# gargatik/Seamless-Through-Breaking-Rethinking-Image-Stitching-for-Optimal-Alignment

Measured on AMD Instinct MI355X. Metric: stitched image-pairs/s at 512x512, higher is better.
Workload: dtype f32 (decoder contractions, PatchEmbed's third conv and the C = 128 block tails: exact 3xbf16 split of both operands, 6 products on the bf16 matrix cores, fp32 accumulate -- error vs fp64 0.83x the fp32 MFMA chain's; everything else fp32); 1 GPU; UDIS-D-shaped 512x512 pairs, batch=1, FlowHomoAdpater.forward(type=test_eval); launch=hipGraph replay, pairs_in_flight=3

## Files before the change

include/stitch_gfx950.h:

```cpp
#ifndef STITCH_GFX950_H
#define STITCH_GFX950_H
#include <stdint.h>
#ifdef __cplusplus
extern "C" {
#endif

typedef struct st_gemm_desc {
    const float* a;
    const float* w;
    float* c;
    const float* bias;
    const float* aux0;
    const float* aux1;
    const float* aux2;
    const float* scale_ptr;
    int32_t M, N, K;
    int32_t H, W, Cin, ldx;
    int32_t kh, kw, sh, sw, ph, pw, Ho, Wo;
    int32_t ldw, ldc, ld_aux0, ld_aux1, ld_aux2;
    int32_t aux0_row_div, aux0_row_mod;
    int32_t act;
    int32_t epi;
    float alpha;
    int32_t batch;
// ... 45 lines not shown
    int32_t ld_res;
    int32_t act;
    int32_t ln;
    float ln_eps;
    int32_t res;
    int32_t res_layer;
} st_chain_layer;
typedef struct st_chain_desc {
    const float* a;
    float* out;
    int32_t lda, ldo, M, nlayers;
    st_chain_layer layer[3];
} st_chain_desc;
int st_linear_chain128(const st_chain_desc* desc, void* stream);
int st_abi_chain_desc_size(void);

typedef struct st_mlp_desc {
    const float* a;
    float* out;
    const float* w1;
    const float* b1;
    const float* w2;
    const float* b2;
    const float* res;
    int32_t lda, ldo, ld_res, M, hidden, ln;
    float ln_eps;
    int32_t reserved;
    const float* wp;
    const float* bp;
    const float* res0;
    int32_t ld_res0, reserved1;
} st_mlp_desc;
int st_mlp128(const st_mlp_desc* desc, void* stream);
int st_abi_mlp_desc_size(void);
int st_mlp128_split3_image_bytes(int32_t hidden, int32_t with_proj, int64_t* bytes);
int st_mlp128_split3_pack(const float* w1, const float* b1, const float* w2, const float* wp, const float* bp, int32_t hidden, void* image,
                          int64_t image_bytes, void* stream);
int st_mlp128_split3(const st_mlp_desc* desc, const void* image, int64_t image_bytes, void* stream);
int st_rowlin128_split3_image_bytes(int32_t N, int64_t* bytes);
int st_rowlin128_split3_pack(const float* w, const float* b, int32_t N, void* image, int64_t image_bytes, void* stream);
int st_rowlin128_split3(const float* a, int32_t lda, float* out, int32_t ldo, int32_t M, int32_t N, int32_t ln, float ln_eps, const void* image,
                        int64_t image_bytes, const float* aux, int32_t ld_aux, int32_t row_div, void* stream);

int st_corr_volume(const float* f1, const float* f2, float* vol, int32_t B, int32_t N1, int32_t N2,
                   int32_t C, void* stream);
int st_corr_volume_both(const float* f1, const float* f2, float* vol12, float* vol21, int32_t B, int32_t N, int32_t C,
                        void* stream);
int st_corr_volume_both_plan(int32_t B, int32_t N, int32_t C, int32_t aligned16);

int st_layernorm(const float* x, int32_t ldx, const float* w, const float* b, float* out, int32_t ldo,
                 int32_t rows, int32_t C, float eps, void* stream);
int st_softmax_rows(float* x, int32_t ld, int32_t rows, int32_t C, void* stream);
int st_l2norm_rows(const float* x, float* out, int32_t rows, int32_t C, void* stream);
int st_maxpool_nhwc(const float* x, float* out, int32_t B, int32_t H, int32_t W, int32_t C, int32_t k,
                    int32_t s, int32_t p, void* stream);
int st_dwconv3x3_residual(const float* x, const float* w, const float* bias, float* out, int32_t B,
                          int32_t H, int32_t W, int32_t C, void* stream);
int st_sine_pe(float* out, int32_t ld, int32_t rows, int32_t dim, const float* coords, int32_t ldc,
               int32_t Wg, int32_t ws, int32_t period, float cscale, float coff, int32_t accumulate,
               void* stream);
int st_attention_small(const float* q, int64_t q_bs, int64_t q_ts, const float* k, int64_t k_bs, int64_t k_ts,
                       const float* v, int64_t v_bs, int64_t v_ts, float* out, int64_t o_bs, int64_t o_ts,
                       int32_t B, int32_t heads, int32_t Nq, int32_t Nk, int32_t D, float scale, void* stream);
int st_attention_kvlds(const float* q, int64_t q_bs, int64_t q_ts, const float* k, int64_t k_bs, int64_t k_ts,
                       const float* v, int64_t v_bs, int64_t v_ts, float* out, int64_t o_bs, int64_t o_ts,
                       int32_t B, int32_t heads, int32_t Nq, int32_t Nk, int32_t D, float scale, void* stream);
int st_window_attention(const float* q, const float* k, const float* v, int64_t bs, int64_t ts,
                        const float* qpad, const float* kpad, const float* vpad, float* out, int64_t o_bs,
                        int64_t o_ts, int32_t B, int32_t H, int32_t W, int32_t heads, int32_t D, int32_t ws,
                        float scale, void* stream);
int st_ccl_softargmax(const float* G, float* out, int32_t ldo, int32_t B, int32_t h, int32_t w, void* stream);
int st_patch_conv1(const float* maps, const float* w36x16, const float* bias, float* out, int32_t M, int32_t H,
                   int32_t W, int32_t Ho, int32_t Wo, void* stream);
int st_patch_conv12(const float* cost_maps, const float* c0_w36x16, const float* c0_b, const float* c2_w32x576,
                    const float* c2_b, float* s2, int32_t M, int32_t H, int32_t W, void* stream);
int st_patch_conv12_planes(const float* cost_maps, const float* c0_w36x16, const float* c0_b, const float* c2_w32x576, const float* c2_b,
                           void* s2_planes, int64_t s2_pstride, int32_t M, int32_t H, int32_t W, void* stream);
int st_copy2d(const float* src, int32_t lds, float* dst, int32_t ldd, int32_t rows, int32_t cols, void* stream);
int st_prep_image(const float* src, float* dst, int32_t B, int32_t C, int32_t H, int32_t W, int32_t ldo,
                  float mul, float div, float sub, void* stream);

int st_latent_pool(const float* scores, int32_t ld_s, const float* tokens, int32_t ld_t, float* z, int32_t pixels,
                   int32_t P, void* stream);

int st_coords_grid(float* out, int32_t B, int32_t H, int32_t W, void* stream);
int st_coords_grid_init(float* out, const float* init, int32_t B, int32_t H, int32_t W, void* stream);
int st_flow_forward_interpolate(const float* src, int32_t src_is_coords_rows, float* out, int32_t B, int32_t H, int32_t W,
                                void* stream);
int st_flow_from_coords(const float* coords1, float* flow4, int32_t ld4, float* dst2, int32_t ld2, int32_t B,
                        int32_t H, int32_t W, void* stream);
int st_flow_encode(const float* coords1, const float* w98, const float* bias, float* out, int32_t ldo, float* flow2,
                   int32_t ld2, int32_t B, int32_t H, int32_t W, int32_t Co, void* stream);
int st_flow_encode_split3(const float* coords1, const float* w98, const float* bias, float* out, int32_t ldo, float* flow2,
                          int32_t ld2, int32_t B, int32_t H, int32_t W, int32_t Co, void* out_planes, int64_t out_pstride,
                          int64_t out_prows, void* flow_planes, int64_t flow_pstride, int64_t flow_prows, int32_t flow_col,
                          void* stream);
int st_cost_lookup(const float* maps, const float* coords, float* out, int32_t ldo, int32_t Nq, int32_t H2,
                   int32_t W2, int32_t r, void* stream);
int st_decoder_token_chain(float* corr, int32_t ld_corr, const float* coords1, const float* kv,
                           const float* const* weights16, int32_t rows, int32_t ntok, void* stream);
int st_convex_upsample(const float* coords1, const float* mask, int32_t ldm, float* out, int32_t B, int32_t H,
                       int32_t W, void* stream);

int st_dlt4(const float* src4x2, const float* motion, float* H, int32_t B, float mscale_x, float mscale_y,
            float div, void* stream);
int st_mat3_sandwich(const float* L, const float* X, const float* R, float* out, int32_t B, int32_t invert,
                     void* stream);
int st_homo_warp(const float* U, const float* theta, float* out, int32_t* idx, int32_t B, int32_t C,
                 int32_t n_ones, int32_t H, int32_t W, int32_t oh, int32_t ow, void* stream);
int st_mesh_bounds(const float* H, float* out4, int32_t B, float width, float height, int32_t gw, int32_t gh,
                   void* stream);
int st_flow_warp(const float* x, const float* flow, const float* mul, float* out, int32_t B, int32_t C,
                 int32_t H, int32_t W, void* stream);
int st_homo_flow_warp(const float* image2, const float* H8, const float* flow, float* out6, float* overlap, float* Hi,
                      int32_t B, int32_t H, int32_t W, void* stream);
int st_resize_bilinear(const float* x, float* out, int32_t planes, int32_t H, int32_t W, int32_t oh, int32_t ow,
                       int32_t align_corners, float div0, float div1, int32_t ndiv, void* stream);
int st_range_map(const float* flow, void* scratch_u64, float* out, int32_t B, int32_t H, int32_t W, void* stream);
int st_occlusion_from_range(const float* range, float* out, int64_t n, int32_t threshold, void* stream);
int st_morph_open(const float* mask, float* out, void* scratch_u8x2, int32_t N, int32_t H, int32_t W,
                  int32_t ksz, void* stream);
int st_eval_finish(float* final6, const float* occ, float* overlap, int32_t B, int32_t H, int32_t W, void* stream);
int st_blend(const float* homo1, const float* homo2, float* fin, const float* occ, float* output2, float* mask1,
             float* mask2, uint8_t* blend, int32_t h, int32_t w, void* stream);
int st_blend_plain(const float* homo1, const float* homo2, const float* fin, float* output2, float* mask1, float* mask2,
                   uint8_t* blend, int32_t h, int32_t w, void* stream);
int st_mean_threshold(const float* x, float* out, int32_t B, int32_t C, int32_t H, int32_t W, float thr,
                      void* stream);
int st_tps_solve_grid(const float* U, const float* source, const float* target, void* work_f64, float* T,
                      float* out, int32_t* idx, int32_t B, int32_t C, int32_t H, int32_t W, int32_t N,
                      int32_t oh, int32_t ow, void* stream);

int st_masked_psnr_ssim(const float* image1, const float* warped, int64_t warped_batch_stride, const float* maskmean,
                        void* partial_f64, double* out_psnr_ssim, int32_t B, int32_t H, int32_t W, void* stream);
int st_channel_mean(const float* x, int64_t batch_stride, float* out, int32_t B, int32_t C, int32_t H, int32_t W,
                    void* stream);

int st_load_rgb8(const void* src_u8_hwc, float* dst_chw, int32_t B, int32_t H, int32_t W, void* stream);

int st_cost_lookup9x9(const float* maps, const float* coords, float* out, int32_t ldo, int32_t Nq, int32_t H2,
                      int32_t W2, void* stream);
int st_grid_sample_blend(const float* x, const float* flow, const float* mul, float* out, int32_t B, int32_t C,
                         int32_t H, int32_t W, void* stream);
int st_morph_open19(const float* mask, float* out, void* scratch_u8x2, int32_t N, int32_t H, int32_t W,
                    void* stream);
int st_patch_embed(const float* cost_maps, const float* const* weights, int32_t ld_f0, const float* pe_bias,
                   float* s1, float* s2, float* s3, float* s4, float* tokens, int32_t M, int32_t H, int32_t W,
                   void* workspace, int64_t workspace_floats, void* stream);
int st_patch_embed_split3(const float* cost_maps, const float* const* weights, int32_t ld_f0, const float* pe_bias, void* s2_planes,
                          int64_t s2_pstride, const void* c4_w_planes, int64_t c4_w_pstride, float* s3, float* s4, float* tokens, int32_t M,
                          int32_t H, int32_t W, const void* tail_image, int64_t tail_image_bytes, void* workspace, int64_t workspace_floats, void* stream);
int st_pe_tail_split3_image_bytes(int64_t* bytes);
int st_pe_tail_split3_pack(const float* w1, int32_t ld1, const float* w2, void* image, int64_t image_bytes, void* stream);
int st_pe_tail_split3(const float* x, const float* tab, int32_t P, const void* image, int64_t image_bytes, const float* b2, const float* gamma,
                      const float* beta, float eps, float* out, int32_t R, void* stream);
int st_gma_attention(const float* inp, int32_t ld_inp, const float* w_qk, float* qk, float* attn, int32_t B,
                     int32_t N, void* workspace, int64_t workspace_floats, void* stream);
int st_gma_aggregate(const float* attn, const float* mf, int32_t ld_mf, const float* w_v, const float* gamma,
                     float* vT, float* out, int32_t ld_out, int32_t B, int32_t N, void* workspace,
                     int64_t workspace_floats, void* stream);
int st_sepconv_gru(float* hxA, float* hxB, int32_t ld, float* zbuf, const float* tab1, const float* tab2,
                   int32_t ld_tab, const float* w_zr1, const float* w_q1, const float* w_zr2, const float* w_q2,
                   int32_t B, int32_t H, int32_t W, void* workspace, int64_t workspace_floats, void* stream);
int st_gma_aggregate_planes(const float* attn, const float* mf, int32_t ld_mf, const float* w_v, const float* gamma, float* vT,
                            float* out, int32_t ld_out, void* out_planes, int64_t out_pstride, int64_t out_prows, int32_t out_col, int32_t B,
                            int32_t N, void* workspace, int64_t workspace_floats, void* stream);
// ... 82 lines not shown
```

seamless-through-breaking-rethinking-image-stitching-for-optimal-alignment_amd/csrc/nn.hip:

```cpp
#include "common.h"
#include "../../include/stitch_gfx950.h"

__global__ __launch_bounds__(256) void layernorm_kernel(const float* __restrict__ x, int ldx, const float* __restrict__ w,
                                                        const float* __restrict__ b, float* __restrict__ out, int ldo,
                                                        int rows, int C, float eps) {
    const int row = (blockIdx.x * 256 + threadIdx.x) >> 6, lane = threadIdx.x & 63;
    if (row >= rows) return;
    const float* xr = x + (size_t)row * ldx;
    float v[16];
    float s = 0.f;
#pragma unroll
    for (int i = 0; i < 16; ++i) {
        const int c = lane + 64 * i;
        v[i] = c < C ? xr[c] : 0.f;
        s += v[i];
    }
    const float mean = wave_sum(s) / (float)C;
    float q = 0.f;
#pragma unroll
    for (int i = 0; i < 16; ++i) {
        const int c = lane + 64 * i;
        const float dlt = c < C ? v[i] - mean : 0.f;
        q += dlt * dlt;
    }
// ... 274 lines not shown
        }
    }
    const float inv = 1.0f / sum;
    float* op = out + b * o_bs + iq * o_ts + h * D;
#pragma unroll
    for (int e = 0; e < D; e += 4)
        *reinterpret_cast<float4*>(op + e) = make_float4(acc[e] * inv, acc[e + 1] * inv, acc[e + 2] * inv, acc[e + 3] * inv);
}

extern "C" int st_attention_small(const float* q, int64_t q_bs, int64_t q_ts, const float* k, int64_t k_bs, int64_t k_ts,
                                  const float* v, int64_t v_bs, int64_t v_ts, float* out, int64_t o_bs, int64_t o_ts,
                                  int32_t B, int32_t heads, int32_t Nq, int32_t Nk, int32_t D, float scale, void* stream) {
    if (!q || !k || !v || !out || B <= 0 || heads <= 0 || Nq <= 0 || Nk <= 0) return ST_EINVAL;
    if (!al16(q) || !al16(k) || !al16(v) || !al16(out) || ((q_bs | q_ts | k_bs | k_ts | v_bs | v_ts | o_bs | o_ts) & 3)) return ST_EINVAL;
    const long total = (long)B * heads * Nq;
    dim3 grid((total + 255) / 256), block(256);
    hipStream_t s = (hipStream_t)stream;
#define LAUNCH_AS(DD) hipLaunchKernelGGL(attention_small_kernel<DD>, grid, block, 0, s, q, q_bs, q_ts, k, k_bs, k_ts, v, \
                                         v_bs, v_ts, out, o_bs, o_ts, B, heads, Nq, Nk, scale)
    if (D == 8) LAUNCH_AS(8); else if (D == 16) LAUNCH_AS(16); else if (D == 32) LAUNCH_AS(32); else return ST_EINVAL;
#undef LAUNCH_AS
    ST_CHECK_LAUNCH();
    return ST_OK;
}

typedef float lp_f32x16 __attribute__((ext_vector_type(16)));

__global__ __launch_bounds__(256) void latent_pool_kernel(const float* __restrict__ scores, int ld_s, const float* __restrict__ tokens,
                                                          int ld_t, float* __restrict__ z, int P) {
    const size_t pix = blockIdx.x;
    const int lane = threadIdx.x & 63, wave = threadIdx.x >> 6;
    const int li = lane & 31, lh = lane >> 5;
    const int ib = wave & 1, jb0 = (wave >> 1) * 2;
    const float* Sp = scores + pix * P * ld_s + ib * 32 + li;
    const float* Tp = tokens + pix * P * ld_t + jb0 * 32 + li;
    const int steps = P >> 1;
    float a[32];
    float mx = -INFINITY;
#pragma unroll
    for (int s = 0; s < 32; ++s) {
        a[s] = s < steps ? Sp[(size_t)(2 * s + lh) * ld_s] : -INFINITY;
        mx = fmaxf(mx, a[s]);
    }
    mx = fmaxf(mx, __shfl_xor(mx, 32, 64));
    float sum = 0.f;
#pragma unroll
    for (int s = 0; s < 32; ++s) { a[s] = __expf(a[s] - mx); sum += a[s]; }
    sum += __shfl_xor(sum, 32, 64);
    const float inv = 1.0f / sum;
    lp_f32x16 acc0, acc1;
#pragma unroll
    for (int r = 0; r < 16; ++r) { acc0[r] = 0.f; acc1[r] = 0.f; }
#pragma unroll
    for (int s0 = 0; s0 < 32; s0 += 8) {
        if (s0 < steps) {
            float b0[8], b1[8];
#pragma unroll
            for (int u = 0; u < 8; ++u) {
                const int tok = min(2 * (s0 + u) + lh, P - 1);
                b0[u] = Tp[(size_t)tok * ld_t];
                b1[u] = Tp[(size_t)tok * ld_t + 32];
            }
#pragma unroll
            for (int u = 0; u < 8; ++u) {
                const float av = a[s0 + u] * inv;
                acc0 = __builtin_amdgcn_mfma_f32_32x32x2f32(av, b0[u], acc0, 0, 0, 0);
                acc1 = __builtin_amdgcn_mfma_f32_32x32x2f32(av, b1[u], acc1, 0, 0, 0);
            }
        }
    }
    float* zp = z + (pix * 64 + ib * 32 + 4 * lh) * 128 + jb0 * 32 + li;
#pragma unroll
    for (int r = 0; r < 16; ++r) {
        const int row = (r & 3) + 8 * (r >> 2);
        zp[(size_t)row * 128] = acc0[r];
        zp[(size_t)row * 128 + 32] = acc1[r];
    }
}

extern "C" int st_latent_pool(const float* scores, int32_t ld_s, const float* tokens, int32_t ld_t, float* z, int32_t pixels,
                              int32_t P, void* stream) {
    if (!scores || !tokens || !z || pixels <= 0 || P <= 0 || (P & 1) || P > 64 || ld_s < 64 || ld_t < 128) return ST_EINVAL;
    hipLaunchKernelGGL(latent_pool_kernel, dim3(pixels), dim3(256), 0, (hipStream_t)stream, scores, ld_s, tokens, ld_t, z, P);
    ST_CHECK_LAUNCH();
    return ST_OK;
}

template <int D>
__global__ __launch_bounds__(256) void attention_kvlds_kernel(const float* __restrict__ q, long q_bs, long q_ts,
                                                              const float* __restrict__ k, long k_bs, long k_ts,
                                                              const float* __restrict__ v, long v_bs, long v_ts,
                                                              float* __restrict__ out, long o_bs, long o_ts, int Nq, int Nk,
                                                              float scale) {
    extern __shared__ __attribute__((aligned(16))) float kv[];
    constexpr int QPT = 2;
    const int h = blockIdx.y, b = blockIdx.z;
    float* Ks = kv;
    float* Vs = kv + (size_t)Nk * D;
    for (int i = threadIdx.x; i < Nk * (D / 4); i += 256) {
        const int j = i / (D / 4), e = (i % (D / 4)) * 4;
        *reinterpret_cast<float4*>(Ks + j * D + e) = *reinterpret_cast<const float4*>(k + b * k_bs + j * k_ts + h * D + e);
        *reinterpret_cast<float4*>(Vs + j * D + e) = *reinterpret_cast<const float4*>(v + b * v_bs + j * v_ts + h * D + e);
    }
    __syncthreads();
    const int iq0 = blockIdx.x * (256 * QPT) + threadIdx.x;
    if (iq0 >= Nq) return;
    float qr[QPT][D], acc[QPT][D], mx[QPT], sum[QPT];
    bool live[QPT];
#pragma unroll
    for (int u = 0; u < QPT; ++u) {
        const int iq = iq0 + 256 * u;
        live[u] = iq < Nq;
        const float* qp = q + b * q_bs + (long)(live[u] ? iq : iq0) * q_ts + h * D;
#pragma unroll
        for (int e = 0; e < D; e += 4) {
            const float4 t = *reinterpret_cast<const float4*>(qp + e);
            qr[u][e] = t.x * scale; qr[u][e + 1] = t.y * scale; qr[u][e + 2] = t.z * scale; qr[u][e + 3] = t.w * scale;
        }
#pragma unroll
        for (int e = 0; e < D; ++e) acc[u][e] = 0.f;
        mx[u] = -INFINITY; sum[u] = 0.f;
    }
    for (int j0 = 0; j0 < Nk; j0 += 8) {
        float s[QPT][8];
#pragma unroll
        for (int jj = 0; jj < 8; ++jj) {
            const int j = j0 + jj;
#pragma unroll
            for (int u = 0; u < QPT; ++u) s[u][jj] = 0.f;
            if (j < Nk) {
#pragma unroll
                for (int e = 0; e < D; e += 4) {
                    const float4 t = *reinterpret_cast<const float4*>(Ks + j * D + e);
#pragma unroll
                    for (int u = 0; u < QPT; ++u) {
                        s[u][jj] = fmaf(qr[u][e], t.x, s[u][jj]); s[u][jj] = fmaf(qr[u][e + 1], t.y, s[u][jj]);
                        s[u][jj] = fmaf(qr[u][e + 2], t.z, s[u][jj]); s[u][jj] = fmaf(qr[u][e + 3], t.w, s[u][jj]);
                    }
                }
            } else {
#pragma unroll
                for (int u = 0; u < QPT; ++u) s[u][jj] = -INFINITY;
            }
        }
#pragma unroll
        for (int u = 0; u < QPT; ++u) {
            float nm = mx[u];
#pragma unroll
            for (int jj = 0; jj < 8; ++jj) nm = fmaxf(nm, s[u][jj]);
            const float corr = __expf(mx[u] - nm);
            mx[u] = nm;
            sum[u] *= corr;
#pragma unroll
            for (int e = 0; e < D; ++e) acc[u][e] *= corr;
#pragma unroll
            for (int jj = 0; jj < 8; ++jj) { s[u][jj] = __expf(s[u][jj] - nm); sum[u] += s[u][jj]; }
        }
#pragma unroll
        for (int jj = 0; jj < 8; ++jj) {
            const int j = j0 + jj;
            if (j < Nk) {
#pragma unroll
                for (int e = 0; e < D; e += 4) {
                    const float4 t = *reinterpret_cast<const float4*>(Vs + j * D + e);
#pragma unroll
                    for (int u = 0; u < QPT; ++u) {
// ... 507 lines not shown
```

seamless-through-breaking-rethinking-image-stitching-for-optimal-alignment_amd/flowformer.py:

```python
from __future__ import annotations

import os

import torch
import torch.nn as nn

from . import ops
from .checkpoint import HP, ParamTree, flat_params, flow_spec
from .homography import pack_conv


SPLIT3 = os.environ.get("ST_SPLIT3", "1") != "0"


def _new(rows, cols, dev, zero=False):
    return (torch.zeros if zero else torch.empty)((rows, cols), device=dev, dtype=torch.float32)


def _planes_copy(p):
    return ops.Planes(p.rows, p.C, None, t=p.t.clone(), c0=p.c0, ncols=p.ncols)


def _keep(trace, **named):
    if trace is None:
# ... 241 lines not shown
            ops.conv_gemm(h, fc2[0], o, bias=fc2[1], aux0=x, epi="add", aux1=extra_res)
        return o

    def _twins(self, t, x, B, H, W, trace=None):
        dev = x.device
        dims, heads, srs, patch = (128, 256), (4, 8), (8, 4), (4, 2)
        for s in range(2):
            C, hd, sr, ps = dims[s], heads[s], srs[s], patch[s]
            H, W = H // ps, W // ps
            N = B * H * W
            e = _new(N, C, dev)
            ops.conv_gemm(x, t[f"pe{s}"][0], e, geom=(B, H * ps, W * ps, ps, ps, ps, ps, 0, 0), bias=t[f"pe{s}"][1])
            x = _new(N, C, dev)
            ops.layernorm(e, t[f"pen{s}"][0], t[f"pen{s}"][1], x, 1e-5)
            L = t[f"l{s}"]
            y = _new(N, C, dev)
            qkv = _new(N, 3 * C, dev)
            if L.get("qkv_s3") is not None:
                ops.rowlin128_split3(x, qkv, L["qkv_s3"], ln_eps=1e-6)
            elif "qkv_ln" in L:
                ops.conv_gemm(x, L["qkv_ln"][0], qkv, bias=L["qkv_ln"][1], ln_eps=1e-6)
            else:
                ops.layernorm(x, L["n1"][0], L["n1"][1], y, 1e-6)
                ops.conv_gemm(y, L["qkv"][0], qkv, bias=L["qkv"][1])
            att = _new(N, C, dev)
            ops.window_attention(qkv[:, :C], qkv[:, C:2 * C], qkv[:, 2 * C:], H * W * 3 * C, 3 * C, *L["pads"], att,
                                 H * W * C, C, B, H, W, hd, C // hd, 7, (C // hd) ** -0.5)
            x2 = self._mlp(att, L["proj"], x, L["n2"], L["fc1"], L["fc2"], 1e-6, fc1_ln=L.get("fc1_ln"), image=L.get("mlp_s3"))
            x3 = _new(N, C, dev)
            ops.dwconv3x3_residual(x2, t[f"peg{s}"][0], t[f"peg{s}"][1], x3, B, H, W, C)
            Gk = t[f"g{s}"]
            ops.layernorm(x3, Gk["n1"][0], Gk["n1"][1], y, 1e-6)
            q = _new(N, C, dev)
            ops.conv_gemm(y, Gk["q"][0], q, bias=Gk["q"][1])
            Hk, Wk = H // sr, W // sr
            Nk = Hk * Wk
            xs = _new(B * Nk, C, dev)
            ops.conv_gemm(y, Gk["sr"][0], xs, geom=(B, H, W, sr, sr, sr, sr, 0, 0), bias=Gk["sr"][1])
            xsn = _new(B * Nk, C, dev)
            ops.layernorm(xs, Gk["srn"][0], Gk["srn"][1], xsn, 1e-5)
            kv = _new(B * Nk, 2 * C, dev)
            ops.conv_gemm(xsn, Gk["kv"][0], kv, bias=Gk["kv"][1])
            ops.attention_kvlds(q, (H * W * C, C), kv[:, :C], (Nk * 2 * C, 2 * C), kv[:, C:], (Nk * 2 * C, 2 * C), att,
                                (H * W * C, C), B, hd, H * W, Nk, C // hd, (C // hd) ** -0.5)
            rec = _record(trace)
            _keep(rec, H=H, W=W, pe=x, lsa=x2, peg=x3)
            x = self._mlp(att, Gk["proj"], x3, Gk["n2"], Gk["fc1"], Gk["fc2"], 1e-6, fc1_ln=Gk.get("fc1_ln"), image=Gk.get("mlp_s3"))
            _keep(rec, gsa=x)
        return x, H, W

    def _patch_embed(self, cost_maps, M, H2, W2):
        pe = self._pk["pe"]
        dev = cost_maps.device
        Hp, Wp = (H2 + 7) // 8 * 8, (W2 + 7) // 8 * 8
        H1, W1, H2p, W2p, h, w = Hp // 2, Wp // 2, Hp // 4, Wp // 4, Hp // 8, Wp // 8
        P = h * w
        key = ("pe_tab", h, w)
        if key not in self._const:
            tab_in = _new(P, 64, dev)
            ops.sine_pe(tab_in, 64, Wg=w, cscale=8.0, coff=4.0)
            tab = _new(P, 128, dev)
            ops.conv_gemm(tab_in, pe["f0"][0][:, 64:], tab, bias=pe["f0"][1])
            self._const[key] = tab
        s3, s4, f = _new(M * P, 64, dev), _new(M * P, 128, dev), _new(M * P, 128, dev)
        if H2 == 64 and W2 == 64 and "c4_s3" in pe:
            CH = 16384
            s2p = ops.Planes(min(M, CH) * 256, 32, dev)
            for m0 in range(0, M, CH):
                m1 = min(M, m0 + CH)
                ops.patch_embed_split3(cost_maps[m0:m1], pe["embed11"], pe["f0"][0].stride(0), self._const[key], s2p, pe["c4_s3"],
                                       s3[m0 * P:m1 * P], s4[m0 * P:m1 * P], f[m0 * P:m1 * P], m1 - m0, H2, W2, tail_image=pe.get("tail_s3"))
            return f, P
        s1 = None if (H2 == 64 and W2 == 64) else _new(M * H1 * W1, 16, dev)
        s2 = _new(M * H2p * W2p, 32, dev)
        ops.patch_embed(cost_maps, pe["embed11"], pe["f0"][0].stride(0), self._const[key], s1, s2, s3, s4, f, M, H2, W2)
        return f, P

    def _latent_input(self, L, tokens, M, P):
        dev = tokens.device
        lat = self._pk["latents"]
        nl = lat.shape[0]
        att = _new(M * nl, 128, dev)
        if nl == 8 and P % 2 == 0 and P <= 64:
            S = _new(M * P, nl * 8, dev)
            ops.conv_gemm(tokens, L["qfold"], S)
            z = _new(M * nl * 8, 128, dev)
            ops.latent_pool(S, tokens, z, M, P)
            ops.conv_gemm(z.view(M * nl, 8 * 128)[:, :128], L["wv_heads"][:16], att[:, :16], batch=8, bsa=128, bsw=16 * 128, bsc=16)
            proj_b = L["proj_b_fold"]
        else:
            qn = _new(nl, 128, dev)
            ops.layernorm(lat, L["n1"][0], L["n1"][1], qn, 1e-5)
            q = _new(nl, 128, dev)
            ops.conv_gemm(qn, L["q"][0], q, bias=L["q"][1])
            kv = _new(M * P, 256, dev)
            ops.conv_gemm(tokens, L["kv"][0], kv, bias=L["kv"][1])
            ops.attention_small(q, (0, 128), kv[:, :128], (P * 256, 256), kv[:, 128:], (P * 256, 256), att, (nl * 128, 128),
                                M, 8, nl, P, 16, 16 ** -0.5)
            proj_b = L["proj"][1]
        x1 = _new(M * nl, 128, dev)
        ops.conv_gemm(att, L["proj"][0], x1, bias=proj_b, aux0=lat, row_mod=nl)
        o = _new(M * nl, 128, dev)
        if L.get("mlp_s3_plain") is not None:
            return ops.mlp128(x1, o, L["f0_ln"][0], L["f0_ln"][1], L["f3"][0], L["f3"][1], ln_eps=1e-5, image=L["mlp_s3_plain"])
        return ops.linear_chain128(x1, o, [dict(w=L["f0_ln"][0], bias=L["f0_ln"][1], act="gelu", ln_eps=1e-5), dict(w=L["f3"][0], bias=L["f3"][1], res=0)])

    def _latent_self(self, L, x, M):
        dev = x.device
        nl = self._pk["latents"].shape[0]
        qkv = _new(M * nl, 384, dev)
        if L.get("qkv_s3") is not None:
            ops.rowlin128_split3(x, qkv, L["qkv_s3"], ln_eps=1e-5)
        else:
            ops.conv_gemm(x, L["qkv_ln"][0], qkv, bias=L["qkv_ln"][1], ln_eps=1e-5)
        att = _new(M * nl, 128, dev)
        ops.attention_small(qkv[:, :128], (nl * 384, 384), qkv[:, 128:256], (nl * 384, 384), qkv[:, 256:], (nl * 384, 384),
                            att, (nl * 128, 128), M, 8, nl, nl, 16, 16 ** -0.5)
        o = _new(M * nl, 128, dev)
        if L.get("mlp_s3") is not None:
            return ops.mlp128(att, o, L["f0_ln"][0], L["f0_ln"][1], L["f3"][0], L["f3"][1], ln_eps=1e-5, proj=(L["proj"][0], L["proj"][1], x), image=L["mlp_s3"])
        return ops.linear_chain128(att, o, [dict(w=L["proj"][0], bias=L["proj"][1], res=x),
                                            dict(w=L["f0_ln"][0], bias=L["f0_ln"][1], act="gelu", ln_eps=1e-5),
                                            dict(w=L["f3"][0], bias=L["f3"][1], res=1)])

    def _vertical(self, V, x, ctx, B, H1, W1, nl, extra_res=None):
        dev = x.device
        N = H1 * W1
        R = B * N * nl
        C, Cc = 128, 64
        Cq = C + Cc
        y = _new(R, C, dev)
        z = _new(B * N, Cq, dev)
        ops.conv_gemm(ctx, V["lctx"][0], z[:, C:], bias=V["lctx"][1])
        ops.sine_pe(z, Cq, Wg=W1, ws=7, period=N, accumulate=C)
        T = _new(B * N, 3 * C, dev)
        ops.conv_gemm(z, V["ltab"][0], T, bias=V["ltab"][1])
        qkv = _new(R, 3 * C, dev)
        if V.get("lqkv_s3") is not None:
            ops.rowlin128_split3(x, qkv, V["lqkv_s3"], ln_eps=1e-5, aux=T, row_div=nl)
        else:
            ops.conv_gemm(x, V["lqkv_ln"][0], qkv, bias=V["lqkv_ln"][1], aux0=T, row_div=nl, ln_eps=1e-5)
        q, k, v = qkv[:, :C], qkv[:, C:2 * C], qkv[:, 2 * C:]
        key = ("lsa_pad", id(V))
        if key not in self._const:
            zp = _new(49, Cq, dev, zero=True)
            ops.sine_pe(zp, Cq, Wg=7, accumulate=True)
            qp, kp = _new(49, C, dev), _new(49, C, dev)
            ops.conv_gemm(zp, V["lq"][0], qp, bias=V["lq"][1])
            ops.conv_gemm(zp, V["lk"][0], kp, bias=V["lk"][1])
            self._const[key] = (qp, kp, V["lv"][1].expand(49, C).contiguous())
        qp, kp, vp = self._const[key]
        att = _new(R, C, dev)
        for b in range(B):
            sl = slice(b * N * nl, (b + 1) * N * nl)
            ops.window_attention(q[sl], k[sl], v[sl], 3 * C, nl * 3 * C, qp, kp, vp, att[sl], C, nl * C, nl, H1, W1, 8, 16, 7,
                                 16 ** -0.5)
        x2 = self._mlp(att, V["lproj"], x, V["ln2"], V["lfc1"], V["lfc2"], 1e-5, fc1_ln=V["lfc1_ln"], image=V.get("lmlp_s3"))
        ops.layernorm(x2, V["gn1"][0], V["gn1"][1], y, 1e-5)
        z = _new(B * N, Cq, dev)
        ops.conv_gemm(ctx, V["gctx"][0], z[:, C:], bias=V["gctx"][1])
        Hk, Wk = H1 // 4, W1 // 4
        Nk = Hk * Wk
        Tkv = _new(B * Nk, 2 * C, dev)
        ops.conv_gemm(z[:, C:], V["gtab"][0], Tkv, geom=(B, H1, W1, 4, 4, 4, 4, 0, 0), bias=V["gtab"][1])
        ops.sine_pe(z, Cq, Wg=W1, period=N, accumulate=C)
        Tq, q = _new(B * N, C, dev), _new(R, C, dev)
        ops.conv_gemm(z, V["gq"][0], Tq, bias=V["gq"][1])
        ops.conv_gemm(y, V["gq"][0][:, :C], q, aux0=Tq, row_div=nl)
        key = ("gsa_kpe", id(V), Hk, Wk)
        if key not in self._const:
            pe_k = _new(Nk, C, dev)
# ... 195 lines not shown
```

seamless-through-breaking-rethinking-image-stitching-for-optimal-alignment_amd/ops.py:

```python
from __future__ import annotations

import ctypes as C

import torch

from ._lib import ChainDesc, GemmDesc, MlpDesc, check, lib
from ._lib import StitchError as StitchErrorBase

ACT = dict(none=0, relu=1, gelu=2, sigmoid=3, tanh=4, lrelu=5)
EPI = dict(store=0, add=1, mul=2, gru=3, axpy=4, zr=5)

assert lib.st_abi_gemm_desc_size() == C.sizeof(GemmDesc), "st_gemm_desc ABI mismatch between header and binding"
assert lib.st_abi_chain_desc_size() == C.sizeof(ChainDesc), "st_chain_desc ABI mismatch between header and binding"
assert lib.st_abi_mlp_desc_size() == C.sizeof(MlpDesc), "st_mlp_desc ABI mismatch between header and binding"


def _stream():
    return C.c_void_p(torch.cuda.current_stream().cuda_stream)


def _p(t):
    if t is None:
        return None
    assert t.is_cuda, "device tensor expected (no CPU fallback)"
# ... 246 lines not shown
    d.ln, d.ln_eps = (1, float(ln_eps)) if ln_eps is not None else (0, 0.0)
    if res is not None:
        assert res.shape == a.shape
        d.res, d.ld_res = res.data_ptr(), _ld(res)
    if proj is not None:
        wp, bp, res0 = proj
        assert wp.shape == (128, 128) and wp.is_contiguous()
        d.wp = wp.data_ptr()
        if bp is not None:
            d.bp = bp.data_ptr()
        if res0 is not None:
            assert res0.shape == a.shape
            d.res0, d.ld_res0 = res0.data_ptr(), _ld(res0)
    if image is not None:
        check(lib.st_mlp128_split3(C.byref(d), C.c_void_p(image.data_ptr()), image.numel(), _stream()), "st_mlp128_split3")
        return out
    check(lib.st_mlp128(C.byref(d), _stream()), "st_mlp128")
    return out


def corr_volume(f1, f2, out):
    B, N1, Cc = f1.shape
    N2 = f2.shape[1]
    check(lib.st_corr_volume(_p(f1), _p(f2), _p(out), B, N1, N2, Cc, _stream()), "st_corr_volume")
    return out


def corr_volume_split3(f1p, f2p, out12, out21, B, N, Cc):
    assert f1p.pstride == f2p.pstride and f1p.rows == f2p.rows
    check(lib.st_corr_volume_split3(C.c_void_p(f1p.ptr()), C.c_void_p(f2p.ptr()), f1p.pstride, f1p.rows, _pc(out12), _pc(out21) if out21 is not None else None,
                                    B, N, Cc, _stream()), "st_corr_volume_split3")
    return out12


def corr_volume_both(f1, f2, out12, out21):
    B, N, Cc = f1.shape
    check(lib.st_corr_volume_both(_p(f1), _p(f2), _pc(out12), _pc(out21), B, N, Cc, _stream()), "st_corr_volume_both")
    return out12, out21


def layernorm(x, w, b, out, eps):
    check(lib.st_layernorm(_p(x), _ld(x), _p(w), _p(b), _p(out), _ld(out), x.shape[0], x.shape[1], eps, _stream()),
          "st_layernorm")
    return out


def softmax_rows(x):
    check(lib.st_softmax_rows(_p(x), _ld(x), x.shape[0], x.shape[1], _stream()), "st_softmax_rows")
    return x


def l2norm_rows(x, out):
    check(lib.st_l2norm_rows(_p(x), _p(out), x.shape[0], x.shape[1], _stream()), "st_l2norm_rows")
    return out


def maxpool(x, out, B, H, W, Cc, k, s, p):
    check(lib.st_maxpool_nhwc(_p(x), _p(out), B, H, W, Cc, k, s, p, _stream()), "st_maxpool_nhwc")
    return out


def dwconv3x3_residual(x, w9c, bias, out, B, H, W, Cc):
    check(lib.st_dwconv3x3_residual(_p(x), _p(w9c), _p(bias), _p(out), B, H, W, Cc, _stream()), "st_dwconv3x3_residual")
    return out


def sine_pe(out, dim, *, coords=None, Wg=0, ws=0, period=0, cscale=1.0, coff=0.0, accumulate=False):
    check(lib.st_sine_pe(_p(out), _ld(out), out.shape[0], dim, _p(coords), _ld(coords) if coords is not None else 0,
                         Wg, ws, period, cscale, coff, int(accumulate), _stream()), "st_sine_pe")
    return out


def attention_small(q, qs, k, ks, v, vs, out, os_, B, heads, Nq, Nk, D, scale):
    check(lib.st_attention_small(_p(q), qs[0], qs[1], _p(k), ks[0], ks[1], _p(v), vs[0], vs[1], _p(out), os_[0], os_[1],
                                 B, heads, Nq, Nk, D, scale, _stream()), "st_attention_small")
    return out


def latent_pool(scores, tokens, z, pixels, P):
    check(lib.st_latent_pool(_p(scores), _ld(scores), _p(tokens), _ld(tokens), _pc(z), pixels, P, _stream()), "st_latent_pool")
    return z


def attention_kvlds(q, qs, k, ks, v, vs, out, os_, B, heads, Nq, Nk, D, scale):
    check(lib.st_attention_kvlds(_p(q), qs[0], qs[1], _p(k), ks[0], ks[1], _p(v), vs[0], vs[1], _p(out), os_[0], os_[1],
                                 B, heads, Nq, Nk, D, scale, _stream()), "st_attention_kvlds")
    return out


def window_attention(q, k, v, bs, ts, qpad, kpad, vpad, out, o_bs, o_ts, B, H, W, heads, D, ws, scale):
    check(lib.st_window_attention(_p(q), _p(k), _p(v), bs, ts, _p(qpad), _p(kpad), _p(vpad), _p(out), o_bs, o_ts, B, H, W,
                                  heads, D, ws, scale, _stream()), "st_window_attention")
    return out


def ccl_softargmax(G, out, B, h, w):
    check(lib.st_ccl_softargmax(_p(G), _p(out), _ld(out), B, h, w, _stream()), "st_ccl_softargmax")
    return out


def patch_conv1(maps, w36x16, bias, out, M, H, W, Ho, Wo):
    check(lib.st_patch_conv1(_pc(maps), _pc(w36x16), _pc(bias), _p(out), M, H, W, Ho, Wo, _stream()), "st_patch_conv1")
    return out


def copy2d(src, dst):
    check(lib.st_copy2d(_p(src), _ld(src), _p(dst), _ld(dst), src.shape[0], src.shape[1], _stream()), "st_copy2d")
    return dst


def prep_image(src, dst, ldo, mul, div, sub):
    B, Cc, H, W = src.shape
    check(lib.st_prep_image(_pc(src), _p(dst), B, Cc, H, W, ldo, mul, div, sub, _stream()), "st_prep_image")
    return dst


def coords_grid(out, B, H, W, init=None):
    if init is None:
        check(lib.st_coords_grid(_p(out), B, H, W, _stream()), "st_coords_grid")
        return
    if tuple(init.shape) != (B, 2, H, W) or init.dtype != torch.float32 or not init.is_contiguous() or init.device != out.device:
        raise ValueError(f"flow_init must be a contiguous float32 [{B}, 2, {H}, {W}] tensor on {out.device}")
    check(lib.st_coords_grid_init(_p(out), _p(init), B, H, W, _stream()), "st_coords_grid_init")


def forward_interpolate(flow, out=None, *, coords_rows=None):
    if coords_rows is None:
        B, two, H, W = flow.shape
        ok = two == 2
    else:
        B, H, W = coords_rows
        ok = tuple(flow.shape) == (B * H * W, 2)
    if not ok or flow.dtype != torch.float32 or not flow.is_contiguous() or not flow.is_cuda:
        raise ValueError("forward_interpolate takes a contiguous float32 cuda tensor [B,2,H1,W1], or coords1 rows [B*H1*W1,2]")
    if out is None:
        out = torch.empty((B, 2, H, W), device=flow.device)
    elif tuple(out.shape) != (B, 2, H, W) or out.dtype != torch.float32 or not out.is_contiguous() or out.device != flow.device:
        raise ValueError(f"out must be a contiguous float32 [{B}, 2, {H}, {W}] tensor on {flow.device}")
    check(lib.st_flow_forward_interpolate(_p(flow), 0 if coords_rows is None else 1, _p(out), B, H, W, _stream()),
          "st_flow_forward_interpolate")
    return out


def flow_from_coords(coords1, flow4, dst2, B, H, W):
    check(lib.st_flow_from_coords(_p(coords1), _p(flow4), _ld(flow4) if flow4 is not None else 0, _p(dst2),
                                  _ld(dst2) if dst2 is not None else 0, B, H, W, _stream()), "st_flow_from_coords")


def flow_encode(coords1, w98, bias, out, flow2, B, H, W):
    check(lib.st_flow_encode(_pc(coords1), _pc(w98), _pc(bias), _p(out), _ld(out), _p(flow2), _ld(flow2) if flow2 is not None else 0,
                             B, H, W, w98.shape[1], _stream()), "st_flow_encode")
    return out


def flow_encode_split3(coords1, w98, bias, out, flow2, B, H, W, out_planes, flow_planes):
    fp, fcol = flow_planes
    check(lib.st_flow_encode_split3(_pc(coords1), _pc(w98), _pc(bias), _p(out), _ld(out), _p(flow2), _ld(flow2), B, H, W, w98.shape[1],
                                    C.c_void_p(out_planes.ptr()), out_planes.pstride, out_planes.rows,
                                    C.c_void_p(fp.t.data_ptr()), fp.pstride, fp.rows, int(fcol), _stream()), "st_flow_encode_split3")
    return out


def cost_lookup(maps, coords, out, Nq, H2, W2, r=4):
    check(lib.st_cost_lookup(_p(maps), _p(coords), _p(out), _ld(out), Nq, H2, W2, r, _stream()), "st_cost_lookup")
    return out

# ... 647 lines not shown
```

Measured before the change: 93.20 pairs/s.

## Fuse latent cross-attention score, pooling and value projection into one kernel

Replaces three launches (score GEMM against folded queries, the softmax latent pool, and the batched per-head value GEMM) with one persistent kernel. It processes two pixels per block, keeps the score matrix and pooled latents in LDS and holds the value weights in registers. This removes the global round trips for the S and z intermediates and two launches. The cost is a large LDS footprint, heavy register use at 512 threads, and a grid capped at 256 blocks, which may limit occupancy.

```diff
diff --git a/include/stitch_gfx950.h b/include/stitch_gfx950.h
--- a/include/stitch_gfx950.h
+++ b/include/stitch_gfx950.h
@@ -151,6 +151,8 @@
 
 int st_latent_pool(const float* scores, int32_t ld_s, const float* tokens, int32_t ld_t, float* z, int32_t pixels,
                    int32_t P, void* stream);
+int st_latent_cross(const float* tokens, int32_t ld_t, const float* qfold, const float* wv_heads, float* att, int32_t ld_att,
+                    int32_t pixels, int32_t P, void* stream);
 
 int st_coords_grid(float* out, int32_t B, int32_t H, int32_t W, void* stream);
 int st_coords_grid_init(float* out, const float* init, int32_t B, int32_t H, int32_t W, void* stream);
diff --git a/seamless-through-breaking-rethinking-image-stitching-for-optimal-alignment_amd/csrc/nn.hip b/seamless-through-breaking-rethinking-image-stitching-for-optimal-alignment_amd/csrc/nn.hip
--- a/seamless-through-breaking-rethinking-image-stitching-for-optimal-alignment_amd/csrc/nn.hip
+++ b/seamless-through-breaking-rethinking-image-stitching-for-optimal-alignment_amd/csrc/nn.hip
@@ -380,6 +380,157 @@
                               int32_t P, void* stream) {
     if (!scores || !tokens || !z || pixels <= 0 || P <= 0 || (P & 1) || P > 64 || ld_s < 64 || ld_t < 128) return ST_EINVAL;
     hipLaunchKernelGGL(latent_pool_kernel, dim3(pixels), dim3(256), 0, (hipStream_t)stream, scores, ld_s, tokens, ld_t, z, P);
+    ST_CHECK_LAUNCH();
+    return ST_OK;
+}
+
+#define LC_LD 132
+#define LC_GROUP_FLOATS (64 * 64 + 64 * LC_LD)
+#define LC_LDS_BYTES ((64 * LC_LD + 2 * LC_GROUP_FLOATS) * 4)
+__global__ __launch_bounds__(512) void latent_cross_kernel(const float* __restrict__ tokens, int ld_t, const float* __restrict__ qfold,
+                                                           const float* __restrict__ wv, float* __restrict__ att, int ld_att,
+                                                           int pixels, int P) {
+    extern __shared__ __attribute__((aligned(16))) float lc_smem[];
+    const int tid = threadIdx.x, lane = tid & 63, wave = __builtin_amdgcn_readfirstlane(tid >> 6);
+    const int li = lane & 31, lh = lane >> 5;
+    const int g = wave >> 2, w = wave & 3;
+    float* Qs = lc_smem;
+    float* Ss = lc_smem + 64 * LC_LD + g * LC_GROUP_FLOATS;
+    float* Zs = Ss + 64 * 64;
+    const int tb = w >> 1, sb = w & 1;
+    const int ib = w & 1, jb0 = (w >> 1) * 2;
+#pragma unroll
+    for (int u = 0; u < 4; ++u) {
+        const int f = u * 512 + tid, rho = f >> 5, c4 = f & 31;
+        *reinterpret_cast<float4*>(Qs + rho * LC_LD + c4 * 4) =
+            *reinterpret_cast<const float4*>(qfold + ((rho & 7) * 8 + (rho >> 3)) * 128 + c4 * 4);
+    }
+    float4 wf[16];
+    {
+        const float* wp = wv + (w * 32 + li) * 128 + 4 * lh;
+#pragma unroll
+        for (int j = 0; j < 16; ++j) wf[j] = *reinterpret_cast<const float4*>(wp + 8 * j);
+    }
+    const bool score_on = tb * 32 < P;
+    const int steps = P >> 1;
+    float4 a[16];
+    auto load_tokens = [&](size_t pix) {
+        const float* p = tokens + (pix * P + min(tb * 32 + li, P - 1)) * ld_t + 4 * lh;
+#pragma unroll
+        for (int j = 0; j < 16; ++j) a[j] = *reinterpret_cast<const float4*>(p + 8 * j);
+    };
+    const int npair = (pixels + 1) >> 1;
+    if (score_on && 2 * (int)blockIdx.x + g < pixels) load_tokens(2 * (size_t)blockIdx.x + g);
+    __syncthreads();
+    for (int pr = blockIdx.x; pr < npair; pr += gridDim.x) {
+        const size_t pix = 2 * (size_t)pr + g;
+        const bool live = pix < (size_t)pixels;
+        if (live && score_on) {
+            const float* qb = Qs + (sb * 32 + li) * LC_LD + 4 * lh;
+            lp_f32x16 acc;
+#pragma unroll
+            for (int r = 0; r < 16; ++r) acc[r] = 0.f;
+            float4 b = *reinterpret_cast<const float4*>(qb);
+#pragma unroll
+            for (int j = 0; j < 16; ++j) {
+                const float4 bn = *reinterpret_cast<const float4*>(qb + 8 * (j + 1 < 16 ? j + 1 : j));
+                acc = __builtin_amdgcn_mfma_f32_32x32x2f32(a[j].x, b.x, acc, 0, 0, 0);
+                acc = __builtin_amdgcn_mfma_f32_32x32x2f32(a[j].y, b.y, acc, 0, 0, 0);
+                acc = __builtin_amdgcn_mfma_f32_32x32x2f32(a[j].z, b.z, acc, 0, 0, 0);
+                acc = __builtin_amdgcn_mfma_f32_32x32x2f32(a[j].w, b.w, acc, 0, 0, 0);
+                b = bn;
+            }
+#pragma unroll
+            for (int r = 0; r < 16; ++r) {
+                const int tok = tb * 32 + (r & 3) + 8 * (r >> 2) + 4 * lh;
+                if (tok < P) Ss[tok * 64 + sb * 32 + li] = acc[r];
+            }
+        }
+        __syncthreads();
+        if (live) {
+            const float* Sp = Ss + ib * 32 + li;
+            const float* Tb = tokens + pix * P * ld_t;
+            const int toff = lh * ld_t + jb0 * 32 + li;
+            float e[32];
+            float mx = -INFINITY;
+#pragma unroll
+            for (int s = 0; s < 32; ++s) {
+                e[s] = s < steps ? Sp[(2 * s + lh) * 64] : -INFINITY;
+                mx = fmaxf(mx, e[s]);
+            }
+            mx = fmaxf(mx, __shfl_xor(mx, 32, 64));
+            float sum = 0.f;
+#pragma unroll
+            for (int s = 0; s < 32; ++s) { e[s] = __expf(e[s] - mx); sum += e[s]; }
+            sum += __shfl_xor(sum, 32, 64);
+            const float inv = 1.0f / sum;
+            lp_f32x16 acc0, acc1;
+#pragma unroll
+            for (int r = 0; r < 16; ++r) { acc0[r] = 0.f; acc1[r] = 0.f; }
+#pragma unroll
+            for (int s0 = 0; s0 < 32; s0 += 8) {
+                if (s0 < steps) {
+                    float b0[8], b1[8];
+#pragma unroll
+                    for (int u = 0; u < 8; ++u) {
+                        const float* tp = Tb + (size_t)(2 * min(s0 + u, steps - 1)) * ld_t;
+                        b0[u] = tp[toff];
+                        b1[u] = tp[toff + 32];
+                    }
+#pragma unroll
+                    for (int u = 0; u < 8; ++u) {
+                        const float av = e[s0 + u] * inv;
+                        acc0 = __builtin_amdgcn_mfma_f32_32x32x2f32(av, b0[u], acc0, 0, 0, 0);
+                        acc1 = __builtin_amdgcn_mfma_f32_32x32x2f32(av, b1[u], acc1, 0, 0, 0);
+                    }
+                }
+            }
+            float* zp = Zs + (ib * 32 + 4 * lh) * LC_LD + jb0 * 32 + li;
+#pragma unroll
+            for (int r = 0; r < 16; ++r) {
+                const int row = (r & 3) + 8 * (r >> 2);
+                zp[row * LC_LD] = acc0[r];
+                zp[row * LC_LD + 32] = acc1[r];
+            }
+            const size_t nxt = pix + 2 * (size_t)gridDim.x;
+            if (score_on && pr + (int)gridDim.x < npair && nxt < (size_t)pixels) load_tokens(nxt);
+        }
+        __syncthreads();
+        if (g == 0) {
+            const float* za = lc_smem + 64 * LC_LD + (li >> 4) * LC_GROUP_FLOATS + 64 * 64 + ((2 * w + ((li >> 3) & 1)) * 8 + (li & 7)) * LC_LD + 4 * lh;
+            lp_f32x16 acc;
+#pragma unroll
+            for (int r = 0; r < 16; ++r) acc[r] = 0.f;
+            float4 zf = *reinterpret_cast<const float4*>(za);
+#pragma unroll
+            for (int j = 0; j < 16; ++j) {
+                const float4 zn = *reinterpret_cast<const float4*>(za + 8 * (j + 1 < 16 ? j + 1 : j));
+                acc = __builtin_amdgcn_mfma_f32_32x32x2f32(zf.x, wf[j].x, acc, 0, 0, 0);
+                acc = __builtin_amdgcn_mfma_f32_32x32x2f32(zf.y, wf[j].y, acc, 0, 0, 0);
+                acc = __builtin_amdgcn_mfma_f32_32x32x2f32(zf.z, wf[j].z, acc, 0, 0, 0);
+                acc = __builtin_amdgcn_mfma_f32_32x32x2f32(zf.w, wf[j].w, acc, 0, 0, 0);
+                zf = zn;
+            }
+            float* op = att + ((size_t)pr * 16 + 4 * lh) * ld_att + w * 32 + li;
+            const bool hi = li >> 4, two = 2 * (size_t)pr + 1 < (size_t)pixels;
+#pragma unroll
+            for (int q = 0; q < 4; ++q) {
+                op[(size_t)q * ld_att] = hi ? acc[4 + q] : acc[q];
+                if (two) op[(size_t)(8 + q) * ld_att] = hi ? acc[12 + q] : acc[8 + q];
+            }
+        }
+    }
+}
+
+extern "C" int st_latent_cross(const float* tokens, int32_t ld_t, const float* qfold, const float* wv_heads, float* att, int32_t ld_att,
+                               int32_t pixels, int32_t P, void* stream) {
+    if (!tokens || !qfold || !wv_heads || !att || pixels <= 0 || P <= 0 || (P & 1) || P > 64 || ld_t < 128 || (ld_t & 3) || ld_att < 128)
+        return ST_EINVAL;
+    if (!al16(tokens) || !al16(qfold) || !al16(wv_heads) || !al16(att)) return ST_EINVAL;
+    const int npair = (pixels + 1) / 2;
+    (void)hipFuncSetAttribute((const void*)latent_cross_kernel, hipFuncAttributeMaxDynamicSharedMemorySize, LC_LDS_BYTES);
+    hipLaunchKernelGGL(latent_cross_kernel, dim3(npair < 256 ? npair : 256), dim3(512), LC_LDS_BYTES, (hipStream_t)stream, tokens, ld_t,
+                       qfold, wv_heads, att, ld_att, pixels, P);
     ST_CHECK_LAUNCH();
     return ST_OK;
 }
diff --git a/seamless-through-breaking-rethinking-image-stitching-for-optimal-alignment_amd/flowformer.py b/seamless-through-breaking-rethinking-image-stitching-for-optimal-alignment_amd/flowformer.py
--- a/seamless-through-breaking-rethinking-image-stitching-for-optimal-alignment_amd/flowformer.py
+++ b/seamless-through-breaking-rethinking-image-stitching-for-optimal-alignment_amd/flowformer.py
@@ -347,11 +347,7 @@
         nl = lat.shape[0]
         att = _new(M * nl, 128, dev)
         if nl == 8 and P % 2 == 0 and P <= 64:
-            S = _new(M * P, nl * 8, dev)
-            ops.conv_gemm(tokens, L["qfold"], S)
-            z = _new(M * nl * 8, 128, dev)
-            ops.latent_pool(S, tokens, z, M, P)
-            ops.conv_gemm(z.view(M * nl, 8 * 128)[:, :128], L["wv_heads"][:16], att[:, :16], batch=8, bsa=128, bsw=16 * 128, bsc=16)
+            ops.latent_cross(tokens, L["qfold"], L["wv_heads"], att, M, P)
             proj_b = L["proj_b_fold"]
         else:
             qn = _new(nl, 128, dev)
diff --git a/seamless-through-breaking-rethinking-image-stitching-for-optimal-alignment_amd/ops.py b/seamless-through-breaking-rethinking-image-stitching-for-optimal-alignment_amd/ops.py
--- a/seamless-through-breaking-rethinking-image-stitching-for-optimal-alignment_amd/ops.py
+++ b/seamless-through-breaking-rethinking-image-stitching-for-optimal-alignment_amd/ops.py
@@ -352,6 +352,12 @@
     return z
 
 
+def latent_cross(tokens, qfold, wv_heads, att, pixels, P):
+    assert tuple(qfold.shape) == (64, 128) and wv_heads.numel() == 8 * 16 * 128, (qfold.shape, wv_heads.shape)
+    check(lib.st_latent_cross(_p(tokens), _ld(tokens), _pc(qfold), _pc(wv_heads), _p(att), _ld(att), pixels, P, _stream()), "st_latent_cross")
+    return att
+
+
 def attention_kvlds(q, qs, k, ks, v, vs, out, os_, B, heads, Nq, Nk, D, scale):
     check(lib.st_attention_kvlds(_p(q), qs[0], qs[1], _p(k), ks[0], ks[1], _p(v), vs[0], vs[1], _p(out), os_[0], os_[1],
                                  B, heads, Nq, Nk, D, scale, _stream()), "st_attention_kvlds")
```

New measurement: 93.29 pairs/s, median of 2. Within noise of the previous version (+0.1%).
